# ZechangSun/QFA

Hardware: AMD Instinct MI355X
Metric: spectra/sec per EM step (higher is better)
Workload: dtype f32

## Files before the change

qfa_amd/csrc/qfa_host.h:

```cpp
#pragma once
#include "qfa_step_kernels.h"
#include "qfa_xdl_kernels.h"
#include "qfa_s12_x.h"

size_t qfa_gx_image_bytes(int KP, int ntiles32);
void qfa_gx_launch(int KP, const qfa_params_t &p, const qfa_batch_t &b, const qfa_tau_t &tau, int B, int Npix, int Nb, int Nh,
                   int ntiles32, const WorkPlan &wp, unsigned char *PGX, const float *SOL, const float *ZS, const float *ZP,
                   float *accum, float *slab, double *slabS, int slab_stride, Scal64 *sc64, unsigned flags, hipStream_t st,
                   bool prep = true);
void qfa_prep_step_launch(int KP, bool pixres, const qfa_params_t &p, const qfa_batch_t &b, const qfa_tau_t &tau, int B, int Npix,
                          int Nb, int Nh, int ntiles32, unsigned char *PFX, unsigned char *P2, float *ZS, float *zero,
                          size_t n_zero, hipStream_t st, unsigned *tick1);

struct GtPlan;
size_t qfa_gt_state_bytes(int KP, int B);
int qfa_gt_items(int KP, int B, int Npix, int max_ranges);
int qfa_gt_ranges(int KP, int B, int Npix, int max_ranges);
void qfa_gt_prep_image(int KP, const qfa_params_t &p, const float *ZP, int Npix, int Nb, int Nh, unsigned char *PGT, hipStream_t st);
void qfa_gt_prep_state(int KP, const float *SOL, int B, int Nh, unsigned char *PST, hipStream_t st);
void qfa_gt_launch(int KP, const qfa_params_t &p, const qfa_batch_t &b, const qfa_tau_t &tau, int B, int Npix, int Nb, int Nh,
                   int max_ranges, const unsigned char *PGT, const unsigned char *PST, const float *ZS, float *accum,
                   float *slab, double *slabS, int slab_stride, Scal64 *sc64, hipStream_t st, int *ranges_out);

size_t qfa_px_image_bytes(int KP, int ntiles32);
// ... 51 lines not shown
        const int nn0 = (ntiles + max_chain - 1) / max_chain, st = (ntiles + nn0 - 1) / nn0;
        return WorkPlan{0, nblk, (ntiles + st - 1) / st, st};
    }
    WorkPlan best{0, nblk, 1, ntiles};
    double best_cost = 1e300;
    for (int full = (nblk / slots) * slots; full >= 0; full -= slots) {
        const int rem = nblk - full;
        for (int n = 1; n <= kMaxSeg; ++n) {
            const bool latency_bound = full == 0 && (long long)rem * n <= slots / 2;
            if (n > 1 && ntiles / n < (latency_bound ? 3 : 8)) break;
            if (n > 8 && !latency_bound) break;
            const int st = (ntiles + n - 1) / n;
            const int nn = (ntiles + st - 1) / st;
            const double rounds_rem = rem ? (double)((long long)rem * nn + slots - 1) / slots : 0.0;
            const double cost = (double)(full / slots) * (ntiles + pro) + (double)(long long)rounds_rem * (st + pro);
            if (cost < best_cost - 1e-9) {
                best_cost = cost;
                best = WorkPlan{full, rem, rem ? nn : 1, rem ? st : ntiles};
            }
            if (!rem) break;
        }
        if (full == 0) break;
    }
    return best;
}

struct Layout {
    int KP, NpixPad, ntiles, Bpad;
    int ntiles32;
    WorkPlan wp1, wp2;
    int spb1;
    WorkPlan wp2x;
    WorkPlan wpp;
    size_t oPF, oPFT, oPFX, oPGX, oPXI, oMOM, oSOL, oNLL, oNBL, oRED, oBG, oZS, oZP, oPST, oISLAB, total;
    int bg_stride;
};

template <int KP>
Layout make_layout_t(int B, int Npix) {
    using C = Cfg<KP>;
    Layout L;
    L.KP = KP;
    L.NpixPad = round_up(Npix, 16);
    L.ntiles = L.NpixPad / 16;
    L.Bpad = round_up(B, 16);
    L.ntiles32 = (Npix + 31) / 32;
    const int NCU = cu_count();
    L.wp2 = plan_work(B, L.ntiles, 4, NCU * (KP == 8 ? QFA_G8_OCC : (KP > 16 ? 1 : 2)));
    L.spb1 = KP <= 16 ? 16 * QFA_P1_NW : 64;
#ifndef QFA_P1_MAX_CHAIN16
#define QFA_P1_MAX_CHAIN16 0
#endif
    L.wp1 = KP <= 16 ? (QFA_P1_NW == 8 ? plan_work(B, L.ntiles32, 1, NCU, 128) : plan_work(B, L.ntiles32, 1, 2 * NCU, 64, QFA_P1_MAX_CHAIN16))
                     : plan_work(B, L.ntiles32, 1, NCU, 64, QFA_P1_MAX_CHAIN);
    size_t o = 0;
    auto take = [&](size_t n) { size_t r = o; o += (n + 63) / 64 * 64; return r; };
    L.oPF = take((size_t)L.ntiles * C::TILE_PF);
    L.oPFT = take((size_t)L.ntiles * C::TILE_PFT);
    L.oPFX = 0;
    L.oPFX = take((size_t)L.ntiles32 * (XCfg<KP>::TILE_B / 4) + 2 * (C::FW + C::PW));
    L.oPGX = 0;
    L.wp2x = WorkPlan{0, 0, 1, 0};
    if constexpr (KP == 8 || KP == 16) {
        L.oPGX = take(qfa_gx_image_bytes(KP, L.ntiles32) / 4);
        L.wp2x = plan_work(B, L.ntiles32, 3, NCU, 64);
    } else if constexpr (QFA_P2_S12 != 0) {
        L.oPGX = take((size_t)L.ntiles32 * (S12<KP>::TILE_B / 4));
        L.wp2x = plan_work(B, L.ntiles32, 3, NCU, 64);
    }
    L.oPXI = 0;
    L.wpp = WorkPlan{0, 0, 1, 0};
    if constexpr (KP <= 16) {
        L.oPXI = take(qfa_px_image_bytes(KP, L.ntiles32) / 4);
        L.wpp = plan_work(B, L.ntiles32, 1, 2 * NCU, 64 * (KP == 16 ? QFA_PX_SPW : QFA_PX_SPW8));
    }
    L.oMOM = take(((size_t)L.Bpad + (size_t)(L.wp1.nseg - 1) * (L.Bpad - (size_t)L.spb1 * (size_t)L.wp1.full)) * C::NMOM);
    L.oSOL = take((size_t)L.Bpad * C::NSOL);
    L.oNLL = take((size_t)L.Bpad);
    L.oNBL = take((size_t)L.Bpad);
    L.oZS = take(4 * (size_t)L.Bpad);
    L.oZP = take(4 * (size_t)L.NpixPad);
    L.oRED = take(2 * 2 * NRED + 2 + sizeof(Scal64) / 4);
    L.oPST = 0;
    if constexpr (KP == 8 || KP == 16) L.oPST = take(qfa_gt_state_bytes(KP, B) / 4);
    L.oISLAB = 0;
    if constexpr (KP == 8 || KP == 16) {
        const size_t rows = (size_t)qfa_gt_ranges(KP, B, Npix, 1 << 30), items8 = 8 * (size_t)qfa_gt_items(KP, B, Npix, 1 << 30);
        const size_t nf = (size_t)Npix * KP + 4 * (size_t)Npix, stride = (nf + 3) / 4 * 4 + 64;
        L.oISLAB = take(rows * stride + (items8 * 3 * 2 + 8) + 2 * ((rows + 31) / 32) * nf + 16);
    }
    L.oBG = 0;
    L.bg_stride = round_up(Npix, 32);
    if constexpr (KP == 32) L.oBG = take(2 * (size_t)round_up(B, 64) * L.bg_stride);
    L.total = o;
    return L;
}

Layout make_layout(int B, int Npix, int Nh) {
    switch (kp_for(Nh)) {
        case 8: return make_layout_t<8>(B, Npix);
        case 16: return make_layout_t<16>(B, Npix);
        default: return make_layout_t<32>(B, Npix);
    }
}

inline int check_batch(const qfa_batch_t &b, int Npix, int Nb) {
    if (!b.delta || !b.error || !b.mask) return QFA_E_NULL;
    const bool fac = b.zq1 || b.pix_ratio;
    if (fac && !(b.zq1 && b.pix_ratio)) return QFA_E_NULL;
    if (fac && b.A_blue) return QFA_E_NULL;
    if (Nb > 0 && !fac && !b.zabs) return QFA_E_NULL;
    if (b.rows && b.A_blue) return QFA_E_NULL;
    if (b.row_stride != 0 && (b.row_stride < (int64_t)Npix || b.row_stride >= (1LL << 31))) return QFA_E_SIZE;
    if (!b.rows && (long long)64 * b.row_stride >= (1LL << 31)) return QFA_E_SIZE;
    return 0;
// ... 13 lines not shown

inline bool pass2_use_xdl(int KP, int B, unsigned flags) {
    (void)B;
    if (flags & QFA_F_PASS2_F32) return false;
    return KP == 16 || KP == 8;
}
inline bool pass2_use_pixres(int KP, int B, int Npix, unsigned flags) {
    if ((KP != 16 && KP != 8) || Npix < 16 || (flags & (QFA_F_PASS2_F32 | QFA_F_S3_FAST))) return false;
    if (flags & QFA_F_PASS2_PIXRES) return true;
    if (flags & QFA_F_PASS2_XDL) return false;
    const int ncu = cu_count();
    if (B >= 96 * ncu) return true;
    if (Npix < 1024) return false;
    return KP == 16 ? B >= 128 : B >= 512;
}

inline int hip_status(hipStream_t st = nullptr, unsigned flags = 0) {
    if (flags & QFA_F_SYNC) {
        hipError_t s = hipStreamSynchronize(st);
        if (s != hipSuccess) { (void)hipGetLastError(); return (int)s; }
    }
    hipError_t e = hipGetLastError();
    return e == hipSuccess ? 0 : (int)e;
}

template <int KP>
void launch_prep(const qfa_params_t &p, const float4 *ZP, int Npix, int Nb, int Nh, const Layout &L, float *PF, float *PFT,
                 hipStream_t st) {
    dim3 blk(64, 4);
    k_prep_pf<KP><<<(L.NpixPad + 3) / 4, blk, 0, st>>>(p.F, p.Psi, p.omega, ZP, Npix, Nb, Nh, L.NpixPad, PF, PFT);
}

template <int KP>
void sum_segments(float *MOM, const Layout &L, int B, hipStream_t st) {
    const WorkPlan &w = L.wp1;
    if (w.rem == 0 || w.nseg <= 1) return;
    const size_t row0 = (size_t)w.full * L.spb1;
    const size_t rows = (size_t)L.Bpad - row0;
    const size_t n4 = rows * Cfg<KP>::NMOM / 4;
    k_sum_segments<<<(unsigned)((n4 + 255) / 256), 256, 0, st>>>(
        reinterpret_cast<float4 *>(MOM + row0 * Cfg<KP>::NMOM),
        reinterpret_cast<const float4 *>(MOM + (size_t)L.Bpad * Cfg<KP>::NMOM), w.nseg, n4);
}

struct ZTables {
    const float4 *ZS, *ZP;
};
inline ZTables launch_zfac(const qfa_params_t &p, const qfa_batch_t &b, const qfa_tau_t &tau, int B, int Nb, const Layout &L,
                           float *ws, hipStream_t st) {
    if (!(b.zq1 && b.pix_ratio) || Nb <= 0) return ZTables{nullptr, nullptr};
    float4 *ZS = reinterpret_cast<float4 *>(ws + L.oZS), *ZP = reinterpret_cast<float4 *>(ws + L.oZP);
    k_zfac_spec<<<(B + 255) / 256, 256, 0, st>>>(b.zq1, b.rows, p, tau, B, ZS);
    k_zfac_pix<<<(Nb + 255) / 256, 256, 0, st>>>(b.pix_ratio, p, tau, Nb, ZP);
    return ZTables{ZS, ZP};
}

template <int KP, bool PREDICT>
void launch_moments(const qfa_params_t &p, const qfa_batch_t &b, const qfa_tau_t &tau, const float *mu, int B, int Npix,
                   int Nb, int Nh, const Layout &L, const ZTables &zt, float *ws, hipStream_t st, bool prep = true) {
    float *MOM = ws + L.oMOM;
    unsigned char *PFX = reinterpret_cast<unsigned char *>(ws + L.oPFX);
    if (prep) {
        if (XCfg<KP>::F16) {
            unsigned *cm = pfx_colmax<KP>(PFX, L.ntiles32);
            (void)hipMemsetAsync(cm, 0, sizeof(unsigned) * XCfg<KP>::NCOL, st);
            k_colmax<KP><<<L.ntiles32, 1024, 0, st>>>(p.F, p.Psi, Npix, Nh, cm);
        }
        k_prep_pfx<KP><<<L.ntiles32, 256, 0, st>>>(p.F, p.Psi, p.omega, PREDICT ? mu : nullptr, zt.ZP, -QFA_LOG2E * tau.offset, Npix, Nb, Nh, PFX);
    }
    constexpr int NW = KP <= 16 ? QFA_P1_NW : 4;
    if (zt.ZS)
        k_moments_x<KP, PREDICT, NW, true><<<L.wp1.items(), 64 * NW, 0, st>>>(p, b, tau, mu, B, L.Bpad, Npix, Nb, L.ntiles32, L.wp1, PFX, zt.ZS, MOM);
    else
        k_moments_x<KP, PREDICT, NW, false><<<L.wp1.items(), 64 * NW, 0, st>>>(p, b, tau, mu, B, L.Bpad, Npix, Nb, L.ntiles32, L.wp1, PFX, nullptr, MOM);
}

inline size_t det_rows_floats(int Npix, int Nb, int Nh) { return (size_t)Npix * Nh + 3 * (size_t)Npix + Nb; }
inline size_t det_row_stride(int Npix, int Nb, int Nh) { return (det_rows_floats(Npix, Nb, Nh) + 3) / 4 * 4 + 64; }
inline size_t det_rows(int B) { return (size_t)((B + 63) / 64); }
constexpr int DET_CHUNK_ROWS = QFA_DET_CHUNK_ROWS;
inline size_t det_chunks(int B) { return (det_rows(B) + DET_CHUNK_ROWS - 1) / DET_CHUNK_ROWS; }
struct DetLayout {
    size_t NF, stride, oS, oPart, bytes;
};
inline DetLayout det_layout(int B, int Npix, int Nb, int Nh) {
    const Layout L = make_layout(B, Npix, Nh);
    size_t items = (size_t)(L.wp2.items() > L.wp2x.items() ? L.wp2.items() : L.wp2x.items());
    if (L.KP == 16 || L.KP == 8) items = std::max(items, 2 * (size_t)qfa_gt_items(L.KP, B, Npix, (int)det_rows(B)));
    DetLayout D;
    D.NF = det_rows_floats(Npix, Nb, Nh);
    D.stride = det_row_stride(Npix, Nb, Nh);
    D.oS = (det_rows(B) * D.stride * sizeof(float) + 15) / 16 * 16;
    D.oPart = D.oS + (items * 4 * 3 * sizeof(double) + 15) / 16 * 16;
    D.bytes = D.oPart + det_chunks(B) * D.NF * sizeof(double);
    return D;
}
inline size_t det_slab_bytes(int B, int Npix, int Nb, int Nh) { return det_layout(B, Npix, Nb, Nh).bytes; }

inline void launch_reduce_slab(const float *slab, const DetLayout &D, int B, int nitemwaves, float *accum, hipStream_t st,
                               int rows = -1) {
    const double *slabS = reinterpret_cast<const double *>(reinterpret_cast<const char *>(slab) + D.oS);
    double *part = reinterpret_cast<double *>(const_cast<char *>(reinterpret_cast<const char *>(slab)) + D.oPart);
    const int nblk = rows >= 0 ? rows : (int)det_rows(B), nch = (nblk + DET_CHUNK_ROWS - 1) / DET_CHUNK_ROWS;
    const unsigned gx = (unsigned)((D.NF + 255) / 256);
    k_reduce_slab_rows<<<dim3(gx, (unsigned)nch), 256, 0, st>>>(slab, nblk, D.NF, D.stride, part);
    k_reduce_slab_fin<<<gx, 256, 0, st>>>(part, slabS, nch, nitemwaves, D.NF, accum);
}

template <int KP>
int run_nll_grad(const qfa_params_t &p, const qfa_batch_t &b, const qfa_tau_t &tau, int B, int Npix, int Nb, int Nh,
                 float *nll, float *accum, float *ws, hipStream_t st, void *const *events, void *slabv, unsigned flags) {
    const Layout L = make_layout_t<KP>(B, Npix);
    float *slab = reinterpret_cast<float *>(slabv);
    DetLayout D{};
    if (slab) D = det_layout(B, Npix, Nb, Nh);
    double *slabS = slab ? reinterpret_cast<double *>(reinterpret_cast<char *>(slab) + D.oS) : nullptr;
    float *PF = ws + L.oPF, *PFT = ws + L.oPFT, *MOM = ws + L.oMOM, *SOL = ws + L.oSOL, *NBL = ws + L.oNBL;
    float *nllbuf = nll ? nll : ws + L.oNLL;
    const size_t accS = (size_t)Npix * Nh + 3 * (size_t)Npix + Nb;
    auto mark = [&](int i) {
        if (events && events[i]) (void)hipEventRecord((hipEvent_t)events[i], st);
    };
    bool pass2_xdl = false;
    if constexpr (KP == 8 || KP == 16) pass2_xdl = pass2_use_xdl(KP, B, flags);
#ifndef QFA_WITH_GFORM
    if constexpr (KP <= 16) { if (flags & QFA_F_S3_FAST) return QFA_E_FLAGS; }
#endif
    mark(0);
    const bool pixres = pass2_xdl && pass2_use_pixres(KP, B, Npix, flags);
    const size_t n_acc = (size_t)Npix * Nh + 3 * (size_t)Npix + Nb + 8;
    ZTables zt{nullptr, nullptr};
    bool fused = false;
    if constexpr (KP == 8 || KP == 16) {
        if (pass2_xdl) {
            fused = true;
            const bool zf = b.zq1 && b.pix_ratio && Nb > 0;
            if (zf) zt.ZS = reinterpret_cast<float4 *>(ws + L.oZS);
            qfa_prep_step_launch(KP, pixres, p, b, tau, B, Npix, Nb, Nh, L.ntiles32, reinterpret_cast<unsigned char *>(ws + L.oPFX),
                                 reinterpret_cast<unsigned char *>(ws + L.oPGX), zf ? ws + L.oZS : nullptr,
                                 (flags & QFA_F_ZERO_ACCUM) ? accum : nullptr, n_acc, st,
                                 reinterpret_cast<unsigned *>(reinterpret_cast<double *>(ws + L.oRED) + 2 * NRED) + 1);
        }
    }
    if (!fused) {
        if (flags & QFA_F_ZERO_ACCUM) (void)hipMemsetAsync(accum, 0, n_acc * sizeof(float), st);
        zt = launch_zfac(p, b, tau, B, Nb, L, ws, st);
        launch_prep<KP>(p, zt.ZP, Npix, Nb, Nh, L, PF, PFT, st);
    }
    mark(1);
    launch_moments<KP, false>(p, b, tau, nullptr, B, Npix, Nb, Nh, L, zt, ws, st, !fused);
    mark(2);
    sum_segments<KP>(MOM, L, B, st);
    constexpr int G = 64 / KP;
    double *red = reinterpret_cast<double *>(ws + L.oRED);
    unsigned *ticket = reinterpret_cast<unsigned *>(red + 2 * NRED);
    Scal64 *sc64 = reinterpret_cast<Scal64 *>(ticket + 2);
    bool solved = false;
    if constexpr (KP == 8 || KP == 16) {
        if (pixres) {
            k_solve<KP, false, true><<<(B + 4 * G - 1) / (4 * G), 256, 0, st>>>(MOM, SOL, nllbuf, NBL, B, Nh, nullptr, nullptr, ticket,
                                                                               reinterpret_cast<unsigned char *>(ws + L.oPST));
            solved = true;
        }
    }
    bool nll_done = false;
    if constexpr (KP == 8 || KP == 16) {
        if (!solved && fused && B <= 2048) {
            k_solve<KP, false, false, true><<<(B + 4 * G - 1) / (4 * G), 256, 0, st>>>(MOM, SOL, nllbuf, NBL, B, Nh, nullptr, nullptr, ticket,
                                                                                      nullptr, accum + accS);
            solved = nll_done = true;
        }
    }
    if (!solved) k_solve<KP, false><<<(B + 4 * G - 1) / (4 * G), 256, 0, st>>>(MOM, SOL, nllbuf, NBL, B, Nh, nullptr, nullptr, ticket);
    const int nred = B <= 2048 ? 1 : (B >= 2048 * NRED ? NRED : (B + 2047) / 2048);
    if (!nll_done) k_reduce_nll<<<nred, 256, 0, st>>>(nllbuf, NBL, B, accum + accS, red, ticket);
    mark(3);
    if (pixres) {
        int ranges = 0;
        float *rowsb = slab;
        DetLayout Dr = D;
        const int maxr = slab ? (int)det_rows(B) : (1 << 30);
        if (!slab) {
            const size_t rows = (size_t)qfa_gt_ranges(KP, B, Npix, maxr), items8 = 8 * (size_t)qfa_gt_items(KP, B, Npix, maxr);
            rowsb = ws + L.oISLAB;
            Dr.NF = det_rows_floats(Npix, Nb, Nh);
            Dr.stride = det_row_stride(Npix, Nb, Nh);
            Dr.oS = (rows * Dr.stride * sizeof(float) + 15) / 16 * 16;
            Dr.oPart = Dr.oS + (items8 * 3 * sizeof(double) + 15) / 16 * 16;
            Dr.bytes = 0;
        }
        double *rowsS = reinterpret_cast<double *>(reinterpret_cast<char *>(rowsb) + Dr.oS);
        qfa_gt_launch(KP, p, b, tau, B, Npix, Nb, Nh, maxr, reinterpret_cast<unsigned char *>(ws + L.oPGX),
                      reinterpret_cast<unsigned char *>(ws + L.oPST), reinterpret_cast<const float *>(zt.ZS), accum, rowsb, rowsS,
                      (int)Dr.stride, sc64, st, &ranges);
        launch_reduce_slab(rowsb, Dr, B, qfa_gt_items(KP, B, Npix, maxr) * 8, accum, st, ranges);
        mark(4);
        return hip_status(st, flags);
    }
    if (pass2_xdl) {
        qfa_gx_launch(KP, p, b, tau, B, Npix, Nb, Nh, L.ntiles32, L.wp2x, reinterpret_cast<unsigned char *>(ws + L.oPGX), SOL,
                      reinterpret_cast<const float *>(zt.ZS), reinterpret_cast<const float *>(zt.ZP), accum, slab, slabS,
                      (int)D.stride, sc64, flags, st, !fused);
        if (slab) launch_reduce_slab(slab, D, B, L.wp2x.items() * 4, accum, st);
        mark(4);
        return hip_status(st, flags);
    }
    if constexpr (KP == 32 && QFA_P2_S12 != 0) {
        float *BG = ws + L.oBG, *GG = BG + (size_t)round_up(B, 64) * L.bg_stride;
        unsigned char *IMG = reinterpret_cast<unsigned char *>(ws + L.oPGX);
        k_prep_s12<KP><<<L.ntiles32, 256, 0, st>>>(p.F, p.Psi, p.omega, zt.ZP, Npix, Nb, Nh, IMG);
        if (b.A_blue)
            k_s12_x<KP, true, false><<<L.wp2x.items(), 256, 0, st>>>(p, b, tau, B, Npix, Nb, Nh, L.ntiles32, L.wp2x, IMG, SOL, BG, GG, L.bg_stride, accum, slab, slabS, (int)D.stride, sc64, nullptr);
        else if (zt.ZS)
            k_s12_x<KP, false, true><<<L.wp2x.items(), 256, 0, st>>>(p, b, tau, B, Npix, Nb, Nh, L.ntiles32, L.wp2x, IMG, SOL, BG, GG, L.bg_stride, accum, slab, slabS, (int)D.stride, sc64, zt.ZS);
        else
            k_s12_x<KP, false, false><<<L.wp2x.items(), 256, 0, st>>>(p, b, tau, B, Npix, Nb, Nh, L.ntiles32, L.wp2x, IMG, SOL, BG, GG, L.bg_stride, accum, slab, slabS, (int)D.stride, sc64, nullptr);
        for (int bh = 0; 16 * bh < Nh; ++bh) {
            if (flags & QFA_F_S3_FAST)
                k_grads_s3<KP, 3><<<L.wp2.items(), 256, 0, st>>>(B, Npix, Nh, L.ntiles, L.wp2, bh, PFT, SOL, BG, GG, L.bg_stride, accum, slab, (int)D.stride);
            else
                k_grads_s3<KP, 6><<<L.wp2.items(), 256, 0, st>>>(B, Npix, Nh, L.ntiles, L.wp2, bh, PFT, SOL, BG, GG, L.bg_stride, accum, slab, (int)D.stride);
        }
        if (slab) launch_reduce_slab(slab, D, B, L.wp2x.items() * 4, accum, st);
        mark(4);
        return hip_status(st, flags);
    }
    auto grads = [&](int bh, float *BG, float *GG) {
        if (b.A_blue)
            k_grads<KP, true, false><<<L.wp2.items(), 256, 0, st>>>(p, b, tau, B, Npix, Nb, Nh, L.ntiles, L.wp2, bh, PFT, SOL, accum, slab, slabS, (int)D.stride, sc64, nullptr, BG, GG, L.bg_stride);
        else if (zt.ZS)
            k_grads<KP, false, true><<<L.wp2.items(), 256, 0, st>>>(p, b, tau, B, Npix, Nb, Nh, L.ntiles, L.wp2, bh, PFT, SOL, accum, slab, slabS, (int)D.stride, sc64, zt.ZS, BG, GG, L.bg_stride);
        else
            k_grads<KP, false, false><<<L.wp2.items(), 256, 0, st>>>(p, b, tau, B, Npix, Nb, Nh, L.ntiles, L.wp2, bh, PFT, SOL, accum, slab, slabS, (int)D.stride, sc64, nullptr, BG, GG, L.bg_stride);
    };
    if constexpr (KP == 32) {
        float *BG = Nh > 16 ? ws + L.oBG : nullptr, *GG = Nh > 16 ? BG + (size_t)round_up(B, 64) * L.bg_stride : nullptr;
        grads(0, BG, GG);
        if (Nh > 16)
            k_grads_s3<KP, 6><<<L.wp2.items(), 256, 0, st>>>(B, Npix, Nh, L.ntiles, L.wp2, 1, PFT, SOL, BG, GG, L.bg_stride, accum, slab, (int)D.stride);
    } else {
    for (int bh = 0; bh < (KP + 15) / 16; ++bh) {
        if (16 * bh >= Nh) break;
        grads(bh, nullptr, nullptr);
    }
    }
    if (slab) launch_reduce_slab(slab, D, B, L.wp2.items() * 4, accum, st);
    mark(4);
    return hip_status(st, flags);
}

template <int KP>
int run_predict(const qfa_params_t &p, const float *mu, const qfa_batch_t &b, const qfa_tau_t &tau, int B, int Npix,
                int Nb, int Nh, float *ll, float *hmean, float *hcov, float *cont, float *unc, float *ws,
                hipStream_t st, void *const *events, unsigned flags) {
    const Layout L = make_layout_t<KP>(B, Npix);
    float *PF = ws + L.oPF, *PFT = ws + L.oPFT, *MOM = ws + L.oMOM, *SOL = ws + L.oSOL;
    auto mark = [&](int i) {
        if (events && events[i]) (void)hipEventRecord((hipEvent_t)events[i], st);
    };
    bool writer_xdl = false;
    if constexpr (KP <= 16 || QFA_P2_S12 != 0) {
        writer_xdl = !(flags & QFA_F_PREDICT_F32);
    }
    mark(0);
    const ZTables zt = launch_zfac(p, b, tau, B, Nb, L, ws, st);
    if (!writer_xdl) launch_prep<KP>(p, nullptr, Npix, Nb, Nh, L, PF, PFT, st);
    launch_moments<KP, true>(p, b, tau, mu, B, Npix, Nb, Nh, L, zt, ws, st);
    mark(1);
    sum_segments<KP>(MOM, L, B, st);
    constexpr int G = 64 / KP;
    k_solve<KP, true><<<(B + 4 * G - 1) / (4 * G), 256, 0, st>>>(MOM, SOL, ll, nullptr, B, Nh, hmean, hcov);
    mark(2);
    if constexpr (KP > 16 && QFA_P2_S12 != 0) {
        if (writer_xdl) {
            unsigned char *IMG = reinterpret_cast<unsigned char *>(ws + L.oPGX);
            k_prep_s12<KP><<<L.ntiles32, 256, 0, st>>>(p.F, mu, p.omega, nullptr, Npix, Nb, Nh, IMG);
            k_predict_x32<KP><<<L.wp2x.items(), 256, 0, st>>>(B, Npix, L.ntiles32, L.wp2x, IMG, SOL, cont, unc);
        }
    }
    if (writer_xdl && KP <= 16)
        qfa_px_launch(KP, p.F, mu, B, Npix, Nh, L.ntiles32, L.wpp, reinterpret_cast<unsigned char *>(ws + L.oPXI), SOL, cont,
                      unc, st);
    else if (!writer_xdl)
        k_predict_out<KP><<<(B + 63) / 64, 256, 0, st>>>(mu, B, Npix, L.ntiles, PFT, SOL, cont, unc);
    mark(3);
    return hip_status(st, flags);
}


}

int qfa_k32_nll_grad(const qfa_params_t &p, const qfa_batch_t &b, const qfa_tau_t &tau, int B, int Npix, int Nb, int Nh,
                     float *nll, float *accum, float *ws, hipStream_t st, void *const *events, void *slab, unsigned flags);
int qfa_k32_predict(const qfa_params_t &p, const float *mu, const qfa_batch_t &b, const qfa_tau_t &tau, int B, int Npix,
                    int Nb, int Nh, float *ll, float *hmean, float *hcov, float *cont, float *unc, float *ws,
                    hipStream_t st, void *const *events, unsigned flags);
```

qfa_amd/csrc/qfa_step_kernels.h:

```cpp
#pragma once
#include <type_traits>

#include "qfa_common.h"
#include "qfa_gt_layout.h"

template <int KP>
__global__ void k_prep_pf(const float *__restrict__ F, const float *__restrict__ Psi,
                          const float *__restrict__ omega, const float4 *__restrict__ ZP, int Npix, int Nb, int Nh,
                          int NpixPad, float *__restrict__ PF, float *__restrict__ PFT) {
    using C = Cfg<KP>;
    const int i = blockIdx.x * blockDim.y + threadIdx.y;
    if (i >= NpixPad) return;
    const bool live = i < Npix;
    float *pft = PFT + (size_t)(i >> 4) * C::TILE_PFT + (i & 15);
    for (int c = threadIdx.x; c < C::NCPL; c += blockDim.x) {
        float v = 0.f;
        int rt = -1;
        if (c < C::FW) {
            if (live && c < Nh) v = F[(size_t)i * Nh + c];
            if (c < KP) rt = c;
        } else if (c < C::PF_PSI) {
            const int pidx = c - C::FW;
            if (pidx < C::KK2) {
                int a = 0;
// ... 72 lines not shown
    }
}

template <int NF4>
struct TileCopy {
    static constexpr int N = (NF4 + 255) / 256;
    static constexpr int NX = N > 3 ? N - 3 : 1;
    static __device__ __forceinline__ bool in(int i, int idx) { return 256 * i + 255 < NF4 || idx < NF4; }
    static __device__ __forceinline__ float4 ld(const float4 *__restrict__ src, int i, int tid) {
        return src[in(i, tid + 256 * i) ? tid + 256 * i : NF4 - 1];
    }
    static __device__ __forceinline__ void load(const float4 *__restrict__ src, int tid, float4 &v0, float4 &v1,
                                                float4 &v2, float4 (&vx)[NX]) {
        v0 = ld(src, 0, tid);
        if (N > 1) v1 = ld(src, 1, tid);
        if (N > 2) v2 = ld(src, 2, tid);
#pragma unroll
        for (int i = 3; i < N; ++i) vx[i - 3] = ld(src, i, tid);
    }
    static __device__ __forceinline__ void store(float4 *dst, int tid, const float4 &v0, const float4 &v1,
                                                 const float4 &v2, const float4 (&vx)[NX]) {
        if (in(0, tid)) dst[tid] = v0;
        if (N > 1 && in(1, tid + 256)) dst[tid + 256] = v1;
        if (N > 2 && in(2, tid + 512)) dst[tid + 512] = v2;
#pragma unroll
        for (int i = 3; i < N; ++i)
            if (in(i, tid + 256 * i)) dst[tid + 256 * i] = vx[i - 3];
    }
};

struct __attribute__((packed, aligned(4))) f4u { float v[4]; };
struct __attribute__((packed, aligned(1))) u4u { unsigned char v[4]; };

static __global__ void k_sum_segments(float4 *__restrict__ mom, const float4 *__restrict__ rest, int nseg, size_t n4) {
    const size_t i = (size_t)blockIdx.x * blockDim.x + threadIdx.x;
    if (i >= n4) return;
    float4 a = mom[i];
    for (int g = 1; g < nseg; ++g) {
        const float4 b = rest[(size_t)(g - 1) * n4 + i];
        a.x += b.x; a.y += b.y; a.z += b.z; a.w += b.w;
    }
    mom[i] = a;
}

#ifndef QFA_SOLVE_OCC4
#define QFA_SOLVE_OCC4 1
#endif
template <int KP, bool PREDICT, bool STATE = false, bool NLLRED = false>
__global__ __launch_bounds__(256, (KP <= 16 && QFA_SOLVE_OCC4) ? 4 : 2) void k_solve(const float *__restrict__ MOM, float *__restrict__ SOL,
                                               float *__restrict__ nll_out, float *__restrict__ nblue_out, int B,
                                               int Nh, float *__restrict__ hmean, float *__restrict__ hcov,
                                               unsigned *__restrict__ ticket = nullptr,
                                               unsigned char *__restrict__ PST = nullptr, float *__restrict__ scal = nullptr) {
    static_assert(!NLLRED || (!PREDICT && !STATE), "NLLRED: the training step of a small batch");
    using C = Cfg<KP>;
    constexpr int G = 64 / KP;
    static_assert(!STATE || ((KP == 16 || KP == 8) && !PREDICT), "state images: N_h <= 16, training step");
    __shared__ __attribute__((aligned(16))) float s_rows[STATE ? 4 * G * C::NSOL : 1];
    if (ticket && blockIdx.x == 0 && threadIdx.x == 0) {
        *ticket = 0u;
        Scal64 *q = reinterpret_cast<Scal64 *>(ticket + 2);
        q->s[0] = 0.0; q->s[1] = 0.0; q->s[2] = 0.0; q->ticket = 0u;
    }
    const int lane = threadIdx.x & 63;
    const int c = lane % KP;
    const int s = (blockIdx.x * (blockDim.x >> 6) + (threadIdx.x >> 6)) * G + lane / KP;
    const bool valid = s < B;
    const float *mom = MOM + (size_t)(valid ? s : B - 1) * C::NMOM;

    constexpr bool VIA_LDS = KP == 32;
    __shared__ __attribute__((aligned(16))) double s_col[VIA_LDS ? 4 * G * KP : 1];
    __shared__ __attribute__((aligned(16))) float s_T[VIA_LDS ? 4 * G * KP * KP : 1];
    double *col = s_col + ((threadIdx.x >> 6) * G + lane / KP) * (VIA_LDS ? KP : 0);
    auto wave_lds_sync = [&]() {
        asm volatile("s_waitcnt lgkmcnt(0)" ::: "memory");
        __builtin_amdgcn_wave_barrier();
    };

    double Cc[KP];
    static_for<KP>([&](auto R) {
        constexpr int r = decltype(R)::value;
        const int a = r < c ? r : c, b = r < c ? c : r;
        Cc[r] = (double)mom[pair_index(a, b, KP)] + (r == c ? 1.0 : 0.0);
    });
    double logdet = 0.0, pprod = 1.0;
    static_for<KP>([&](auto JJ) {
        constexpr int jj = decltype(JJ)::value;
        if constexpr (VIA_LDS) {
            if (c == jj) static_for<KP>([&](auto R) { col[decltype(R)::value] = Cc[decltype(R)::value]; });
            wave_lds_sync();
        }
        const double piv = VIA_LDS ? col[jj] : group_bcast<KP>(Cc[jj], jj);
        pprod *= piv;
        if ((jj & 7) == 7 || jj == KP - 1) {
            logdet += log(pprod);
            pprod = 1.0;
        }
        const double ip = 1.0 / piv;
        const double rjc = (c == jj) ? ip : Cc[jj] * ip;
        const double keep = (c == jj) ? 0.0 : 1.0;
        static_for<KP>([&](auto I) {
            constexpr int i = decltype(I)::value;
            if constexpr (i != jj) {
                const double cij = VIA_LDS ? col[i] : group_bcast<KP>(Cc[i], jj);
                Cc[i] = fma(-cij, rjc, Cc[i] * keep);
            }
        });
        Cc[jj] = rjc;
        if constexpr (VIA_LDS) wave_lds_sync();
        __builtin_amdgcn_sched_barrier(0);
    });
    const double bc = (double)mom[C::MOM_B + c];
    double y = 0.0;
    if constexpr (VIA_LDS) {
        col[c] = bc;
        wave_lds_sync();
    }
    static_for<KP>([&](auto R) {
        constexpr int r = decltype(R)::value;
        y += Cc[r] * (VIA_LDS ? col[r] : group_bcast<KP>(bc, r));
    });
    double quad = bc * y;
#pragma unroll
    for (int o = KP / 2; o >= 1; o >>= 1) quad += __shfl_xor(quad, o, KP);
    const float *sc = mom + C::MOM_S;
    const double nll = 0.5 * ((double)sc[0] - quad + (double)sc[2] * (double)QFA_LOG2PI + (double)sc[1] + logdet);
    if (valid && c == 0) {
        nll_out[s] = (float)nll;
        if (nblue_out) nblue_out[s] = sc[3];
    }

    float *sol = STATE ? s_rows + ((threadIdx.x >> 6) * G + lane / KP) * C::NSOL : SOL + (size_t)(valid ? s : 0) * C::NSOL;
    if (valid) {
        sol[c] = (float)y;
        static_for<KP>([&](auto R) {
            constexpr int r = decltype(R)::value;
            if (r <= c) sol[C::SOL_CI + pair_index(r, c, KP)] = (float)(r == c ? Cc[r] : 2.0 * Cc[r]);
        });
    }
    if (PREDICT) {
        if (valid && c < Nh) {
            hmean[(size_t)s * Nh + c] = (float)y;
            static_for<KP>([&](auto R) {
                constexpr int r = decltype(R)::value;
                if (r < Nh) hcov[((size_t)s * Nh + c) * Nh + r] = (float)Cc[r];
            });
        }
        return;
    }
    float Tc[KP];
    const float *momT = mom;
    if constexpr (VIA_LDS) asm volatile("" : "+v"(momT));
    static_for<KP>([&](auto R) {
        constexpr int r = decltype(R)::value;
        const int a = r < c ? r : c, b = r < c ? c : r;
        Tc[r] = momT[C::MOM_T + pair_index(a, b, KP)];
    });
    float Zr[KP];
    static_for<KP>([&](auto Bq) { Zr[decltype(Bq)::value] = 0.f; });
    double pc = (double)mom[C::MOM_B2 + c];
    if constexpr (VIA_LDS) {
        float *Tl = s_T + ((threadIdx.x >> 6) * G + lane / KP) * KP * KP;
        wave_lds_sync();
        static_for<KP>([&](auto M) { Tl[decltype(M)::value * KP + c] = Tc[decltype(M)::value]; });
        col[c] = y;
        wave_lds_sync();
        static_for<KP>([&](auto M) {
            constexpr int m = decltype(M)::value;
            pc -= (double)Tc[m] * col[m];
        });
        __builtin_amdgcn_sched_barrier(0);
        static_for<KP>([&](auto M) {
            constexpr int m = decltype(M)::value;
            const float cm = (float)Cc[m];
            static_for<KP / 4>([&](auto Bq) {
                constexpr int b = 4 * decltype(Bq)::value;
                const float4 t = *reinterpret_cast<const float4 *>(Tl + m * KP + b);
                Zr[b] = fmaf(cm, t.x, Zr[b]);
                Zr[b + 1] = fmaf(cm, t.y, Zr[b + 1]);
                Zr[b + 2] = fmaf(cm, t.z, Zr[b + 2]);
                Zr[b + 3] = fmaf(cm, t.w, Zr[b + 3]);
            });
            static_for<KP>([&](auto Bq) { pin(Zr[decltype(Bq)::value]); });
            asm volatile("" ::: "memory");
            __builtin_amdgcn_sched_barrier(0);
        });
    } else {
        static_for<KP>([&](auto M) {
            constexpr int m = decltype(M)::value;
            const float cm = (float)Cc[m];
            static_for<KP>([&](auto Bq) {
                constexpr int b = decltype(Bq)::value;
                Zr[b] = fmaf(cm, group_bcast<KP>(Tc[m], b), Zr[b]);
            });
            static_for<KP>([&](auto Bq) { pin(Zr[decltype(Bq)::value]); });
            __builtin_amdgcn_sched_barrier(0);
        });
    }
    if constexpr (!VIA_LDS) {
        static_for<KP>([&](auto M) {
            constexpr int m = decltype(M)::value;
            pc -= (double)Tc[m] * group_bcast<KP>(y, m);
        });
    }
    if (valid) {
        static_for<KP>([&](auto Bq) {
            constexpr int b = decltype(Bq)::value;
            sol[C::SOL_Z + c * KP + b] = Zr[b];
        });
        sol[C::SOL_P + c] = (float)pc;
    }
    if constexpr (STATE) {
        __syncthreads();
#pragma unroll
        for (int q = 0; q < (4 * G) / 16; ++q) {
            const int grp = (int)blockIdx.x * ((4 * G) / 16) + q;
            if (16 * grp < B)
                build_state<KP>(s_rows + q * 16 * C::NSOL, 16 * grp, B, Nh, PST + (size_t)grp * GTT<KP>::STATE_B, (int)threadIdx.x);
        }
    }
    if constexpr (NLLRED) {
        __shared__ double sh[2][4];
        __shared__ bool last;
        __threadfence();
        __syncthreads();
        if (threadIdx.x == 0) last = atomicAdd(ticket + 1, 1u) == (unsigned)gridDim.x - 1u;
        __syncthreads();
        if (!last) return;
        __threadfence();
        double a = 0.0, nb = 0.0;
        for (int q = threadIdx.x; q < B; q += 256) {
            a += (double)__hip_atomic_load(nll_out + q, __ATOMIC_RELAXED, __HIP_MEMORY_SCOPE_AGENT);
            nb += __hip_atomic_load(nblue_out + q, __ATOMIC_RELAXED, __HIP_MEMORY_SCOPE_AGENT) > 0.f ? 1.0 : 0.0;
        }
        for (int o = 32; o >= 1; o >>= 1) {
            a += __shfl_xor(a, o);
            nb += __shfl_xor(nb, o);
        }
        const int w = threadIdx.x >> 6;
        if ((threadIdx.x & 63) == 0) { sh[0][w] = a; sh[1][w] = nb; }
        __syncthreads();
        if (threadIdx.x == 0) {
            double ta = 0.0, tb = 0.0;
            for (int i = 0; i < 4; ++i) { ta += sh[0][i]; tb += sh[1][i]; }
            scal[3] += (float)tb;
            scal[4] += (float)ta;
            scal[5] += (float)B;
        }
    }
}

constexpr int NRED = 32;
static __global__ __launch_bounds__(256) void k_reduce_nll(const float *__restrict__ nll, const float *__restrict__ nblue,
                                                           int B, float *__restrict__ scal, double *__restrict__ part,
                                                           unsigned *__restrict__ ticket) {
    __shared__ double sh[2][4];
    __shared__ bool last;
    const int per = (B + (int)gridDim.x - 1) / (int)gridDim.x, s0 = blockIdx.x * per, s1 = min(B, s0 + per);
    double a = 0.0, nb = 0.0;
    for (int s = s0 + threadIdx.x; s < s1; s += 256) {
        a += (double)nll[s];
        nb += nblue[s] > 0.f ? 1.0 : 0.0;
    }
    for (int o = 32; o >= 1; o >>= 1) {
        a += __shfl_xor(a, o);
        nb += __shfl_xor(nb, o);
    }
    const int w = threadIdx.x >> 6;
    if ((threadIdx.x & 63) == 0) { sh[0][w] = a; sh[1][w] = nb; }
    __syncthreads();
    if (threadIdx.x == 0) {
        double ta = 0.0, tb = 0.0;
        for (int i = 0; i < 4; ++i) { ta += sh[0][i]; tb += sh[1][i]; }
        part[blockIdx.x] = ta;
        part[NRED + blockIdx.x] = tb;
        __threadfence();
        last = atomicAdd(ticket, 1u) == (unsigned)gridDim.x - 1u;
        if (last) {
            __threadfence();
            ta = 0.0; tb = 0.0;
// ... 579 lines not shown

#if QFA_ABL == 7
    if (blk == 300 && lane == 0 && wv == 0 && seg < 4) {
        for (int i = 0; i < 16; ++i) qfa_dbg_stamps[seg * 16 + i] = st_t[i];
    }
#endif
    if (!active) {
        if (det && lane == 0 && bhalf == 0) {
            double *q = slabS + ((size_t)blockIdx.x * 4 + wv) * 3;
            q[0] = 0.0; q[1] = 0.0; q[2] = 0.0;
        } else if (!det && bhalf == 0) {
            scal64_commit(sc64, 0.0, 0.0, 0.0, gridDim.x * 4u, accS);
        }
        return;
    }
    for (int o = 32; o >= 1; o >>= 1) {
        s_tau0 += __shfl_xor(s_tau0, o);
        s_c0 += __shfl_xor(s_c0, o);
        s_beta += __shfl_xor(s_beta, o);
    }
    if (lane == 0 && bhalf == 0) {
        if (det) {
            double *q = slabS + ((size_t)blockIdx.x * 4 + wv) * 3;
            q[0] = s_tau0; q[1] = s_c0; q[2] = s_beta;
        } else {
            scal64_commit(sc64, s_tau0, s_c0, s_beta, gridDim.x * 4u, accS);
        }
    }
}

#ifndef QFA_DET_CHUNK_ROWS
#define QFA_DET_CHUNK_ROWS 32
#endif
static __global__ __launch_bounds__(256) void k_reduce_slab_rows(const float *__restrict__ slab, int nblk, size_t NF,
                                                                 size_t stride, double *__restrict__ part) {
    const size_t j = (size_t)blockIdx.x * 256 + threadIdx.x;
    if (j >= NF) return;
    const int r0 = blockIdx.y * QFA_DET_CHUNK_ROWS, r1 = min(nblk, r0 + QFA_DET_CHUNK_ROWS);
    const float *q = slab + (size_t)r0 * stride + j;
    double a = 0.0;
    int r = r0;
    for (; r + 8 <= r1; r += 8, q += 8 * stride) {
        const float v0 = q[0], v1 = q[stride], v2 = q[2 * stride], v3 = q[3 * stride], v4 = q[4 * stride],
                    v5 = q[5 * stride], v6 = q[6 * stride], v7 = q[7 * stride];
        a += (double)v0; a += (double)v1; a += (double)v2; a += (double)v3;
        a += (double)v4; a += (double)v5; a += (double)v6; a += (double)v7;
    }
    for (; r < r1; ++r, q += stride) a += (double)q[0];
    part[(size_t)blockIdx.y * NF + j] = a;
}
static __global__ __launch_bounds__(256) void k_reduce_slab_fin(const double *__restrict__ part,
                                                                const double *__restrict__ slabS, int nch,
                                                                int nitemwaves, size_t NF, float *__restrict__ accum) {
    const size_t j = (size_t)blockIdx.x * 256 + threadIdx.x;
    if (j < NF) {
        double a = 0.0;
        for (int c = 0; c < nch; ++c) a += part[(size_t)c * NF + j];
        accum[j] += (float)a;
    }
    __shared__ double sh[3][256];
    if (blockIdx.x == 0) {
        const int per = (nitemwaves + 255) / 256, q0 = threadIdx.x * per, q1 = min(nitemwaves, q0 + per);
        double a0 = 0.0, a1 = 0.0, a2 = 0.0;
        for (int q = q0; q < q1; ++q) {
            a0 += slabS[(size_t)q * 3 + 0];
            a1 += slabS[(size_t)q * 3 + 1];
            a2 += slabS[(size_t)q * 3 + 2];
        }
        sh[0][threadIdx.x] = a0; sh[1][threadIdx.x] = a1; sh[2][threadIdx.x] = a2;
        __syncthreads();
        if (threadIdx.x < 3) {
            double a = 0.0;
            for (int t = 0; t < 256; ++t) a += sh[threadIdx.x][t];
            accum[NF + threadIdx.x] += (float)a;
        }
    }
}

template <int KP>
__global__ __launch_bounds__(256) void k_predict_out(const float *__restrict__ mu, int B, int Npix, int ntiles,
                                                     const float *__restrict__ PFT, const float *__restrict__ SOL,
                                                     float *__restrict__ cont, float *__restrict__ unc) {
    using C = Cfg<KP>;
    constexpr int KF = KP / 4, KQ = C::KK2 / 4;
    const int lane = threadIdx.x & 63;
    const int s0 = (blockIdx.x * (blockDim.x >> 6) + (threadIdx.x >> 6)) * 16;
    if (s0 >= B) return;
    const int lo = lane & 15, g = lane >> 4;
    float yA[KF], qA[KQ];
    {
// ... 29 lines not shown
```

Before: 33.50 million.

## Fuse segment sum and NLL/slab reductions into solve and single-pass kernels

Removes the separate k_sum_segments launch by having each solve block first sum its own split-segment moment rows, with blocks processed in reverse order. The NLL reduction becomes a per-block partial published to a buffer, followed by last-block finalization, and it now also runs on the pixres path. The two-kernel slab reduction becomes one kernel with per-column tickets (zeroed inside solve) so the last chunk block finalizes. The non-LDS Z accumulation now stages T through LDS with float4 reads instead of group broadcasts. The aim is fewer launches and less serialization, at the cost of atomics, ticket bookkeeping and more LDS use.

Measured after the change: 33.55 million (median of 6 runs). No clear change (+0.2%).

```diff
diff --git a/qfa_amd/csrc/qfa_host.h b/qfa_amd/csrc/qfa_host.h
--- a/qfa_amd/csrc/qfa_host.h
+++ b/qfa_amd/csrc/qfa_host.h
@@ -107,7 +107,7 @@
     int spb1;
     WorkPlan wp2x;
     WorkPlan wpp;
-    size_t oPF, oPFT, oPFX, oPGX, oPXI, oMOM, oSOL, oNLL, oNBL, oRED, oBG, oZS, oZP, oPST, oISLAB, total;
+    size_t oPF, oPFT, oPFX, oPGX, oPXI, oMOM, oSOL, oNLL, oNBL, oRED, oBG, oZS, oZP, oPST, oISLAB, oNLLP, oSTK, total;
     int bg_stride;
 };
 
@@ -156,6 +156,8 @@
     L.oZS = take(4 * (size_t)L.Bpad);
     L.oZP = take(4 * (size_t)L.NpixPad);
     L.oRED = take(2 * 2 * NRED + 2 + sizeof(Scal64) / 4);
+    L.oNLLP = take(2 * 2 * (size_t)((B + 256 / KP - 1) / (256 / KP)));
+    L.oSTK = take(((KP + 4) * (size_t)Npix + 255) / 256 + 1);
     L.oPST = 0;
     if constexpr (KP == 8 || KP == 16) L.oPST = take(qfa_gt_state_bytes(KP, B) / 4);
     L.oISLAB = 0;
@@ -235,15 +237,11 @@
 }
 
 template <int KP>
-void sum_segments(float *MOM, const Layout &L, int B, hipStream_t st) {
+SegSum seg_sum(const Layout &L) {
     const WorkPlan &w = L.wp1;
-    if (w.rem == 0 || w.nseg <= 1) return;
+    if (w.rem == 0 || w.nseg <= 1) return SegSum{0, 1, 0, 0};
     const size_t row0 = (size_t)w.full * L.spb1;
-    const size_t rows = (size_t)L.Bpad - row0;
-    const size_t n4 = rows * Cfg<KP>::NMOM / 4;
-    k_sum_segments<<<(unsigned)((n4 + 255) / 256), 256, 0, st>>>(
-        reinterpret_cast<float4 *>(MOM + row0 * Cfg<KP>::NMOM),
-        reinterpret_cast<const float4 *>(MOM + (size_t)L.Bpad * Cfg<KP>::NMOM), w.nseg, n4);
+    return SegSum{(int)row0, w.nseg, (size_t)L.Bpad * Cfg<KP>::NMOM, ((size_t)L.Bpad - row0) * Cfg<KP>::NMOM};
 }
 
 struct ZTables {
@@ -300,14 +298,14 @@
 }
 inline size_t det_slab_bytes(int B, int Npix, int Nb, int Nh) { return det_layout(B, Npix, Nb, Nh).bytes; }
 
-inline void launch_reduce_slab(const float *slab, const DetLayout &D, int B, int nitemwaves, float *accum, hipStream_t st,
-                               int rows = -1) {
+inline int slab_tickets(size_t NF) { return (int)((NF + 255) / 256); }
+inline void launch_reduce_slab(const float *slab, const DetLayout &D, int B, int nitemwaves, float *accum, unsigned *tick,
+                               hipStream_t st, int rows = -1) {
     const double *slabS = reinterpret_cast<const double *>(reinterpret_cast<const char *>(slab) + D.oS);
     double *part = reinterpret_cast<double *>(const_cast<char *>(reinterpret_cast<const char *>(slab)) + D.oPart);
     const int nblk = rows >= 0 ? rows : (int)det_rows(B), nch = (nblk + DET_CHUNK_ROWS - 1) / DET_CHUNK_ROWS;
-    const unsigned gx = (unsigned)((D.NF + 255) / 256);
-    k_reduce_slab_rows<<<dim3(gx, (unsigned)nch), 256, 0, st>>>(slab, nblk, D.NF, D.stride, part);
-    k_reduce_slab_fin<<<gx, 256, 0, st>>>(part, slabS, nch, nitemwaves, D.NF, accum);
+    const unsigned gx = (unsigned)slab_tickets(D.NF);
+    k_reduce_slab<<<dim3(gx, (unsigned)nch), 256, 0, st>>>(slab, nblk, D.NF, D.stride, part, slabS, nitemwaves, accum, tick);
 }
 
 template <int KP>
@@ -353,28 +351,29 @@
     mark(1);
     launch_moments<KP, false>(p, b, tau, nullptr, B, Npix, Nb, Nh, L, zt, ws, st, !fused);
     mark(2);
-    sum_segments<KP>(MOM, L, B, st);
+    const SegSum seg = seg_sum<KP>(L);
     constexpr int G = 64 / KP;
+    unsigned *stk = reinterpret_cast<unsigned *>(ws + L.oSTK);
+    const int nstk = slab_tickets(det_rows_floats(Npix, Nb, Nh));
+    double *nllp = reinterpret_cast<double *>(ws + L.oNLLP);
     double *red = reinterpret_cast<double *>(ws + L.oRED);
     unsigned *ticket = reinterpret_cast<unsigned *>(red + 2 * NRED);
     Scal64 *sc64 = reinterpret_cast<Scal64 *>(ticket + 2);
-    bool solved = false;
-    if constexpr (KP == 8 || KP == 16) {
-        if (pixres) {
-            k_solve<KP, false, true><<<(B + 4 * G - 1) / (4 * G), 256, 0, st>>>(MOM, SOL, nllbuf, NBL, B, Nh, nullptr, nullptr, ticket,
-                                                                               reinterpret_cast<unsigned char *>(ws + L.oPST));
-            solved = true;
-        }
-    }
+    const unsigned nsb = (unsigned)((B + 4 * G - 1) / (4 * G));
     bool nll_done = false;
     if constexpr (KP == 8 || KP == 16) {
-        if (!solved && fused && B <= 2048) {
-            k_solve<KP, false, false, true><<<(B + 4 * G - 1) / (4 * G), 256, 0, st>>>(MOM, SOL, nllbuf, NBL, B, Nh, nullptr, nullptr, ticket,
-                                                                                      nullptr, accum + accS);
-            solved = nll_done = true;
-        }
-    }
-    if (!solved) k_solve<KP, false><<<(B + 4 * G - 1) / (4 * G), 256, 0, st>>>(MOM, SOL, nllbuf, NBL, B, Nh, nullptr, nullptr, ticket);
+        if (pixres)
+            k_solve<KP, false, true, true><<<nsb, 256, 0, st>>>(MOM, seg, SOL, nllbuf, NBL, B, Nh, nullptr, nullptr, ticket,
+                                                               reinterpret_cast<unsigned char *>(ws + L.oPST), accum + accS, nllp,
+                                                               stk, nstk);
+        else if (fused)
+            k_solve<KP, false, false, true><<<nsb, 256, 0, st>>>(MOM, seg, SOL, nllbuf, NBL, B, Nh, nullptr, nullptr, ticket, nullptr,
+                                                                accum + accS, nllp, stk, nstk);
+        nll_done = fused;
+    }
+    if (!nll_done)
+        k_solve<KP, false><<<nsb, 256, 0, st>>>(MOM, seg, SOL, nllbuf, NBL, B, Nh, nullptr, nullptr, ticket, nullptr, nullptr, nullptr,
+                                                stk, nstk);
     const int nred = B <= 2048 ? 1 : (B >= 2048 * NRED ? NRED : (B + 2047) / 2048);
     if (!nll_done) k_reduce_nll<<<nred, 256, 0, st>>>(nllbuf, NBL, B, accum + accS, red, ticket);
     mark(3);
@@ -396,7 +395,7 @@
         qfa_gt_launch(KP, p, b, tau, B, Npix, Nb, Nh, maxr, reinterpret_cast<unsigned char *>(ws + L.oPGX),
                       reinterpret_cast<unsigned char *>(ws + L.oPST), reinterpret_cast<const float *>(zt.ZS), accum, rowsb, rowsS,
                       (int)Dr.stride, sc64, st, &ranges);
-        launch_reduce_slab(rowsb, Dr, B, qfa_gt_items(KP, B, Npix, maxr) * 8, accum, st, ranges);
+        launch_reduce_slab(rowsb, Dr, B, qfa_gt_items(KP, B, Npix, maxr) * 8, accum, stk, st, ranges);
         mark(4);
         return hip_status(st, flags);
     }
@@ -404,7 +403,7 @@
         qfa_gx_launch(KP, p, b, tau, B, Npix, Nb, Nh, L.ntiles32, L.wp2x, reinterpret_cast<unsigned char *>(ws + L.oPGX), SOL,
                       reinterpret_cast<const float *>(zt.ZS), reinterpret_cast<const float *>(zt.ZP), accum, slab, slabS,
                       (int)D.stride, sc64, flags, st, !fused);
-        if (slab) launch_reduce_slab(slab, D, B, L.wp2x.items() * 4, accum, st);
+        if (slab) launch_reduce_slab(slab, D, B, L.wp2x.items() * 4, accum, stk, st);
         mark(4);
         return hip_status(st, flags);
     }
@@ -424,7 +423,7 @@
             else
                 k_grads_s3<KP, 6><<<L.wp2.items(), 256, 0, st>>>(B, Npix, Nh, L.ntiles, L.wp2, bh, PFT, SOL, BG, GG, L.bg_stride, accum, slab, (int)D.stride);
         }
-        if (slab) launch_reduce_slab(slab, D, B, L.wp2x.items() * 4, accum, st);
+        if (slab) launch_reduce_slab(slab, D, B, L.wp2x.items() * 4, accum, stk, st);
         mark(4);
         return hip_status(st, flags);
     }
@@ -447,7 +446,7 @@
         grads(bh, nullptr, nullptr);
     }
     }
-    if (slab) launch_reduce_slab(slab, D, B, L.wp2.items() * 4, accum, st);
+    if (slab) launch_reduce_slab(slab, D, B, L.wp2.items() * 4, accum, stk, st);
     mark(4);
     return hip_status(st, flags);
 }
@@ -470,9 +469,8 @@
     if (!writer_xdl) launch_prep<KP>(p, nullptr, Npix, Nb, Nh, L, PF, PFT, st);
     launch_moments<KP, true>(p, b, tau, mu, B, Npix, Nb, Nh, L, zt, ws, st);
     mark(1);
-    sum_segments<KP>(MOM, L, B, st);
     constexpr int G = 64 / KP;
-    k_solve<KP, true><<<(B + 4 * G - 1) / (4 * G), 256, 0, st>>>(MOM, SOL, ll, nullptr, B, Nh, hmean, hcov);
+    k_solve<KP, true><<<(B + 4 * G - 1) / (4 * G), 256, 0, st>>>(MOM, seg_sum<KP>(L), SOL, ll, nullptr, B, Nh, hmean, hcov);
     mark(2);
     if constexpr (KP > 16 && QFA_P2_S12 != 0) {
         if (writer_xdl) {
diff --git a/qfa_amd/csrc/qfa_step_kernels.h b/qfa_amd/csrc/qfa_step_kernels.h
--- a/qfa_amd/csrc/qfa_step_kernels.h
+++ b/qfa_amd/csrc/qfa_step_kernels.h
@@ -128,27 +128,27 @@
 struct __attribute__((packed, aligned(4))) f4u { float v[4]; };
 struct __attribute__((packed, aligned(1))) u4u { unsigned char v[4]; };
 
-static __global__ void k_sum_segments(float4 *__restrict__ mom, const float4 *__restrict__ rest, int nseg, size_t n4) {
-    const size_t i = (size_t)blockIdx.x * blockDim.x + threadIdx.x;
-    if (i >= n4) return;
-    float4 a = mom[i];
-    for (int g = 1; g < nseg; ++g) {
-        const float4 b = rest[(size_t)(g - 1) * n4 + i];
-        a.x += b.x; a.y += b.y; a.z += b.z; a.w += b.w;
-    }
-    mom[i] = a;
+struct SegSum {
+    int row0, nseg;
+    size_t rest, stride;
+};
+
+__device__ __forceinline__ void slab_publish(double *p, double v) {
+    __hip_atomic_store(p, v, __ATOMIC_RELAXED, __HIP_MEMORY_SCOPE_AGENT);
 }
 
 #ifndef QFA_SOLVE_OCC4
 #define QFA_SOLVE_OCC4 1
 #endif
 template <int KP, bool PREDICT, bool STATE = false, bool NLLRED = false>
-__global__ __launch_bounds__(256, (KP <= 16 && QFA_SOLVE_OCC4) ? 4 : 2) void k_solve(const float *__restrict__ MOM, float *__restrict__ SOL,
+__global__ __launch_bounds__(256, (KP <= 16 && QFA_SOLVE_OCC4) ? 4 : 2) void k_solve(float *__restrict__ MOM, SegSum seg, float *__restrict__ SOL,
                                                float *__restrict__ nll_out, float *__restrict__ nblue_out, int B,
                                                int Nh, float *__restrict__ hmean, float *__restrict__ hcov,
                                                unsigned *__restrict__ ticket = nullptr,
-                                               unsigned char *__restrict__ PST = nullptr, float *__restrict__ scal = nullptr) {
-    static_assert(!NLLRED || (!PREDICT && !STATE), "NLLRED: the training step of a small batch");
+                                               unsigned char *__restrict__ PST = nullptr, float *__restrict__ scal = nullptr,
+                                               double *__restrict__ part = nullptr, unsigned *__restrict__ tk_zero = nullptr,
+                                               int n_tk_zero = 0) {
+    static_assert(!NLLRED || (!PREDICT && KP <= 16), "NLLRED: the training step, N_h <= 16");
     using C = Cfg<KP>;
     constexpr int G = 64 / KP;
     static_assert(!STATE || ((KP == 16 || KP == 8) && !PREDICT), "state images: N_h <= 16, training step");
@@ -158,15 +158,36 @@
         Scal64 *q = reinterpret_cast<Scal64 *>(ticket + 2);
         q->s[0] = 0.0; q->s[1] = 0.0; q->s[2] = 0.0; q->ticket = 0u;
     }
+    const int lb = (int)gridDim.x - 1 - (int)blockIdx.x;
+    if (tk_zero && blockIdx.x == 0)
+        for (int i = threadIdx.x; i < n_tk_zero; i += blockDim.x) tk_zero[i] = 0u;
+    {
+        const int sb0 = lb * 4 * G;
+        if (seg.nseg > 1 && sb0 >= seg.row0) {
+            const int n4 = (min(4 * G, B - sb0) * C::NMOM) / 4;
+            float4 *m4 = reinterpret_cast<float4 *>(MOM + (size_t)sb0 * C::NMOM);
+            const float4 *r4 = reinterpret_cast<const float4 *>(MOM + seg.rest + (size_t)(sb0 - seg.row0) * C::NMOM);
+            const size_t st4 = seg.stride / 4;
+            for (int i = threadIdx.x; i < n4; i += blockDim.x) {
+                float4 a = m4[i];
+                for (int g = 1; g < seg.nseg; ++g) {
+                    const float4 b = r4[(size_t)(g - 1) * st4 + i];
+                    a.x += b.x; a.y += b.y; a.z += b.z; a.w += b.w;
+                }
+                m4[i] = a;
+            }
+            __syncthreads();
+        }
+    }
     const int lane = threadIdx.x & 63;
     const int c = lane % KP;
-    const int s = (blockIdx.x * (blockDim.x >> 6) + (threadIdx.x >> 6)) * G + lane / KP;
+    const int s = (lb * (blockDim.x >> 6) + (threadIdx.x >> 6)) * G + lane / KP;
     const bool valid = s < B;
     const float *mom = MOM + (size_t)(valid ? s : B - 1) * C::NMOM;
 
     constexpr bool VIA_LDS = KP == 32;
     __shared__ __attribute__((aligned(16))) double s_col[VIA_LDS ? 4 * G * KP : 1];
-    __shared__ __attribute__((aligned(16))) float s_T[VIA_LDS ? 4 * G * KP * KP : 1];
+    __shared__ __attribute__((aligned(16))) float s_T[(VIA_LDS || (!STATE && !PREDICT)) ? 4 * G * KP * KP : 1];
     double *col = s_col + ((threadIdx.x >> 6) * G + lane / KP) * (VIA_LDS ? KP : 0);
     auto wave_lds_sync = [&]() {
         asm volatile("s_waitcnt lgkmcnt(0)" ::: "memory");
@@ -224,6 +245,55 @@
     if (valid && c == 0) {
         nll_out[s] = (float)nll;
         if (nblue_out) nblue_out[s] = sc[3];
+    }
+    if constexpr (NLLRED) {
+        __shared__ double sh[2][4 * G > 4 ? 4 * G : 4];
+        __shared__ bool last;
+        const int q = (threadIdx.x >> 6) * G + lane / KP;
+        if (c == 0) {
+            sh[0][q] = valid ? (double)(float)nll : 0.0;
+            sh[1][q] = valid && sc[3] > 0.f ? 1.0 : 0.0;
+        }
+        __syncthreads();
+        const int nblk = (int)gridDim.x;
+        if (threadIdx.x == 0) {
+            double ta = 0.0, tb = 0.0;
+            for (int i = 0; i < 4 * G; ++i) { ta += sh[0][i]; tb += sh[1][i]; }
+            slab_publish(part + lb, ta);
+            slab_publish(part + nblk + lb, tb);
+            asm volatile("s_waitcnt vmcnt(0)" ::: "memory");
+            last = atomicAdd(ticket + 1, 1u) == (unsigned)nblk - 1u;
+        }
+        __syncthreads();
+        if (last) {
+        const int per = (nblk + 255) / 256, q0 = threadIdx.x * per, q1 = min(nblk, q0 + per);
+        double a = 0.0, nb = 0.0;
+        for (int i = q0; i < q1; i += 8) {
+            double va[8], vb[8];
+#pragma unroll
+            for (int k = 0; k < 8; ++k) {
+                va[k] = i + k < q1 ? __hip_atomic_load(part + i + k, __ATOMIC_RELAXED, __HIP_MEMORY_SCOPE_AGENT) : 0.0;
+                vb[k] = i + k < q1 ? __hip_atomic_load(part + nblk + i + k, __ATOMIC_RELAXED, __HIP_MEMORY_SCOPE_AGENT) : 0.0;
+            }
+#pragma unroll
+            for (int k = 0; k < 8; ++k) { a += va[k]; nb += vb[k]; }
+        }
+        __syncthreads();
+        for (int o = 32; o >= 1; o >>= 1) {
+            a += __shfl_xor(a, o);
+            nb += __shfl_xor(nb, o);
+        }
+        const int w = threadIdx.x >> 6;
+        if ((threadIdx.x & 63) == 0) { sh[0][w] = a; sh[1][w] = nb; }
+        __syncthreads();
+        if (threadIdx.x == 0) {
+            double ta = 0.0, tb = 0.0;
+            for (int i = 0; i < 4; ++i) { ta += sh[0][i]; tb += sh[1][i]; }
+            scal[3] += (float)tb;
+            scal[4] += (float)ta;
+            scal[5] += (float)B;
+        }
+        }
     }
 
     float *sol = STATE ? s_rows + ((threadIdx.x >> 6) * G + lane / KP) * C::NSOL : SOL + (size_t)(valid ? s : 0) * C::NSOL;
@@ -282,14 +352,22 @@
             __builtin_amdgcn_sched_barrier(0);
         });
     } else {
+        float *Tl = STATE ? sol + C::SOL_Z : s_T + ((threadIdx.x >> 6) * G + lane / KP) * KP * KP;
+        static_for<KP>([&](auto M) { Tl[decltype(M)::value * KP + c] = Tc[decltype(M)::value]; });
+        wave_lds_sync();
         static_for<KP>([&](auto M) {
             constexpr int m = decltype(M)::value;
             const float cm = (float)Cc[m];
-            static_for<KP>([&](auto Bq) {
-                constexpr int b = decltype(Bq)::value;
-                Zr[b] = fmaf(cm, group_bcast<KP>(Tc[m], b), Zr[b]);
+            static_for<KP / 4>([&](auto Bq) {
+                constexpr int b = 4 * decltype(Bq)::value;
+                const float4 t = *reinterpret_cast<const float4 *>(Tl + m * KP + b);
+                Zr[b] = fmaf(cm, t.x, Zr[b]);
+                Zr[b + 1] = fmaf(cm, t.y, Zr[b + 1]);
+                Zr[b + 2] = fmaf(cm, t.z, Zr[b + 2]);
+                Zr[b + 3] = fmaf(cm, t.w, Zr[b + 3]);
             });
             static_for<KP>([&](auto Bq) { pin(Zr[decltype(Bq)::value]); });
+            asm volatile("" ::: "memory");
             __builtin_amdgcn_sched_barrier(0);
         });
     }
@@ -310,38 +388,9 @@
         __syncthreads();
 #pragma unroll
         for (int q = 0; q < (4 * G) / 16; ++q) {
-            const int grp = (int)blockIdx.x * ((4 * G) / 16) + q;
+            const int grp = lb * ((4 * G) / 16) + q;
             if (16 * grp < B)
                 build_state<KP>(s_rows + q * 16 * C::NSOL, 16 * grp, B, Nh, PST + (size_t)grp * GTT<KP>::STATE_B, (int)threadIdx.x);
-        }
-    }
-    if constexpr (NLLRED) {
-        __shared__ double sh[2][4];
-        __shared__ bool last;
-        __threadfence();
-        __syncthreads();
-        if (threadIdx.x == 0) last = atomicAdd(ticket + 1, 1u) == (unsigned)gridDim.x - 1u;
-        __syncthreads();
-        if (!last) return;
-        __threadfence();
-        double a = 0.0, nb = 0.0;
-        for (int q = threadIdx.x; q < B; q += 256) {
-            a += (double)__hip_atomic_load(nll_out + q, __ATOMIC_RELAXED, __HIP_MEMORY_SCOPE_AGENT);
-            nb += __hip_atomic_load(nblue_out + q, __ATOMIC_RELAXED, __HIP_MEMORY_SCOPE_AGENT) > 0.f ? 1.0 : 0.0;
-        }
-        for (int o = 32; o >= 1; o >>= 1) {
-            a += __shfl_xor(a, o);
-            nb += __shfl_xor(nb, o);
-        }
-        const int w = threadIdx.x >> 6;
-        if ((threadIdx.x & 63) == 0) { sh[0][w] = a; sh[1][w] = nb; }
-        __syncthreads();
-        if (threadIdx.x == 0) {
-            double ta = 0.0, tb = 0.0;
-            for (int i = 0; i < 4; ++i) { ta += sh[0][i]; tb += sh[1][i]; }
-            scal[3] += (float)tb;
-            scal[4] += (float)ta;
-            scal[5] += (float)B;
         }
     }
 }
@@ -987,30 +1036,34 @@
 #ifndef QFA_DET_CHUNK_ROWS
 #define QFA_DET_CHUNK_ROWS 32
 #endif
-static __global__ __launch_bounds__(256) void k_reduce_slab_rows(const float *__restrict__ slab, int nblk, size_t NF,
-                                                                 size_t stride, double *__restrict__ part) {
+static __global__ __launch_bounds__(256) void k_reduce_slab(const float *__restrict__ slab, int nblk, size_t NF, size_t stride,
+                                                            double *__restrict__ part, const double *__restrict__ slabS,
+                                                            int nitemwaves, float *__restrict__ accum, unsigned *__restrict__ tick) {
     const size_t j = (size_t)blockIdx.x * 256 + threadIdx.x;
-    if (j >= NF) return;
-    const int r0 = blockIdx.y * QFA_DET_CHUNK_ROWS, r1 = min(nblk, r0 + QFA_DET_CHUNK_ROWS);
-    const float *q = slab + (size_t)r0 * stride + j;
-    double a = 0.0;
-    int r = r0;
-    for (; r + 8 <= r1; r += 8, q += 8 * stride) {
-        const float v0 = q[0], v1 = q[stride], v2 = q[2 * stride], v3 = q[3 * stride], v4 = q[4 * stride],
-                    v5 = q[5 * stride], v6 = q[6 * stride], v7 = q[7 * stride];
-        a += (double)v0; a += (double)v1; a += (double)v2; a += (double)v3;
-        a += (double)v4; a += (double)v5; a += (double)v6; a += (double)v7;
-    }
-    for (; r < r1; ++r, q += stride) a += (double)q[0];
-    part[(size_t)blockIdx.y * NF + j] = a;
-}
-static __global__ __launch_bounds__(256) void k_reduce_slab_fin(const double *__restrict__ part,
-                                                                const double *__restrict__ slabS, int nch,
-                                                                int nitemwaves, size_t NF, float *__restrict__ accum) {
-    const size_t j = (size_t)blockIdx.x * 256 + threadIdx.x;
+    const int nch = (int)gridDim.y;
+    if (j < NF) {
+        const int r0 = blockIdx.y * QFA_DET_CHUNK_ROWS, r1 = min(nblk, r0 + QFA_DET_CHUNK_ROWS);
+        const float *q = slab + (size_t)r0 * stride + j;
+        double a = 0.0;
+        int r = r0;
+        for (; r + 8 <= r1; r += 8, q += 8 * stride) {
+            const float v0 = q[0], v1 = q[stride], v2 = q[2 * stride], v3 = q[3 * stride], v4 = q[4 * stride],
+                        v5 = q[5 * stride], v6 = q[6 * stride], v7 = q[7 * stride];
+            a += (double)v0; a += (double)v1; a += (double)v2; a += (double)v3;
+            a += (double)v4; a += (double)v5; a += (double)v6; a += (double)v7;
+        }
+        for (; r < r1; ++r, q += stride) a += (double)q[0];
+        slab_publish(part + (size_t)blockIdx.y * NF + j, a);
+    }
+    __shared__ bool last;
+    asm volatile("s_waitcnt vmcnt(0)" ::: "memory");
+    __syncthreads();
+    if (threadIdx.x == 0) last = atomicAdd(tick + blockIdx.x, 1u) == (unsigned)nch - 1u;
+    __syncthreads();
+    if (!last) return;
     if (j < NF) {
         double a = 0.0;
-        for (int c = 0; c < nch; ++c) a += part[(size_t)c * NF + j];
+        for (int c = 0; c < nch; ++c) a += __hip_atomic_load(part + (size_t)c * NF + j, __ATOMIC_RELAXED, __HIP_MEMORY_SCOPE_AGENT);
         accum[j] += (float)a;
     }
     __shared__ double sh[3][256];
```
